# leoelm/Bayesian_inference_for_NN

Measured on NVIDIA B200. Metric: posterior_grad_evals_per_s, higher is better.
Workload: dtype f32 (tensor-core products on two int8 fixed-point slices per operand, kind::i8, exact int32 accumulate; f32 everywhere else)

## Files before the change

bayesian_inference_for_nn_b200/csrc/tc_fused.cuh:

```cuda
#pragma once
#include "tc_layer2.cuh"

namespace pyb {

constexpr int TF_THREADS = 384;
template <int CP> struct TfCfg {
  static constexpr int STAGES = 5;
  static constexpr int W2_BYTES = 2 * 256 * CP * 4;
  static constexpr int ZX_BYTES = 2 * CP * 128 * 4;
  static constexpr int SMEM = STAGES * TP_STAGE_BYTES + 1024  + 1024  + 2048  +
                              128  + W2_BYTES + ZX_BYTES;
  static constexpr int SMEM_I8 = SMEM + 4096;
};
__device__ __forceinline__ void tc_ld_16x256b_x4_raw(uint32_t taddr, uint32_t* r) {
  asm volatile(
      "tcgen05.ld.sync.aligned.16x256b.x4.b32 "
      "{%0, %1, %2, %3, %4, %5, %6, %7, %8, %9, %10, %11, %12, %13, %14, %15}, [%16];"
      : "=r"(r[0]), "=r"(r[1]), "=r"(r[2]), "=r"(r[3]), "=r"(r[4]), "=r"(r[5]), "=r"(r[6]), "=r"(r[7]), "=r"(r[8]),
        "=r"(r[9]), "=r"(r[10]), "=r"(r[11]), "=r"(r[12]), "=r"(r[13]), "=r"(r[14]), "=r"(r[15])
      : "r"(taddr)
      : "memory");
}
__device__ __forceinline__ void tc_mma_i8_pair(uint32_t tmem_d, uint64_t adesc, uint64_t bdesc, uint32_t idesc,
                                               uint32_t accumulate) {
  asm volatile(
      "{\n"
      ".reg .pred p;\n"
      "setp.ne.b32 p, %4, 0;\n"
      "tcgen05.mma.cta_group::2.kind::i8 [%0], %1, %2, %3, p;\n"
      "}\n" ::"r"(tmem_d),
      "l"(adesc), "l"(bdesc), "r"(idesc), "r"(accumulate)
      : "memory");
}
__device__ __forceinline__ void slice4_i8(const float* d, float zq, uint32_t& hw, uint32_t& lw) {
  constexpr float M = 12582912.0f;
  uint32_t hb[4], lb[4];
#pragma unroll
  for (int r = 0; r < 4; ++r) {
    const float t = fmaf(d[r], zq, M);
    const float h = t - M;
    const float e = fmaf(d[r], zq, -h);
    const float u = fmaf(e, 254.0f, M);
    hb[r] = __float_as_uint(t);
    lb[r] = __float_as_uint(u);
  }
  hw = __byte_perm(__byte_perm(hb[0], hb[1], 0x0040), __byte_perm(hb[2], hb[3], 0x0040), 0x5410);
  lw = __byte_perm(__byte_perm(lb[0], lb[1], 0x0040), __byte_perm(lb[2], lb[3], 0x0040), 0x5410);
}

__device__ __forceinline__ void tc_ld_16x256b_x4(uint32_t taddr, float* v) {
  uint32_t r[16];
  asm volatile(
      "tcgen05.ld.sync.aligned.16x256b.x4.b32 "
      "{%0, %1, %2, %3, %4, %5, %6, %7, %8, %9, %10, %11, %12, %13, %14, %15}, [%16];"
      : "=r"(r[0]), "=r"(r[1]), "=r"(r[2]), "=r"(r[3]), "=r"(r[4]), "=r"(r[5]), "=r"(r[6]), "=r"(r[7]), "=r"(r[8]),
        "=r"(r[9]), "=r"(r[10]), "=r"(r[11]), "=r"(r[12]), "=r"(r[13]), "=r"(r[14]), "=r"(r[15])
      : "r"(taddr)
      : "memory");
#pragma unroll
  for (int i = 0; i < 16; ++i) v[i] = __uint_as_float(r[i]);
}
template <int CP>
__device__ __forceinline__ int w2_slot(int h, int c) {
  return ((((h >> 3) * 2 + (h & 1)) * (CP / 4) + (c >> 2)) * 4 + ((h >> 1) & 3)) * 4 + (c & 3);
}
__device__ __forceinline__ void split_pair(float x0, float x1, uint32_t& hw, uint32_t& lw) {
  const __nv_bfloat162 hp = __floats2bfloat162_rn(x0, x1);
  hw = *reinterpret_cast<const uint32_t*>(&hp);
  const __nv_bfloat162 lp = __floats2bfloat162_rn(x0 - __uint_as_float(hw << 16), x1 - __uint_as_float(hw & 0xffff0000u));
  lw = *reinterpret_cast<const uint32_t*>(&lp);
}

template <int CP, bool FWD, int I8 = 0>
__global__ void __cluster_dims__(2, 1, 1) __launch_bounds__(TF_THREADS, 1)
tc_g1_layer2_fused(const __grid_constant__ CUtensorMap tmA_hi, const __grid_constant__ CUtensorMap tmA_lo,
                   const __grid_constant__ CUtensorMap tmB_hi, const __grid_constant__ CUtensorMap tmB_lo,
                   const TcGemmParams p, const Layer2Params l2) {
  constexpr int STAGES = TfCfg<CP>::STAGES;
  extern __shared__ uint8_t smem_raw[];
  uint8_t* smem = smem_raw + ((1024u - (smem_u32(smem_raw) & 1023u)) & 1023u);
  uint8_t* stage_base = smem;
  uint64_t* bars = (uint64_t*)(smem + STAGES * TP_STAGE_BYTES);
  uint64_t* full_bar = bars;
  uint64_t* empty_bar = bars + STAGES;
  uint64_t* tmem_full = bars + 2 * STAGES;
  uint64_t* tmem_empty = bars + 2 * STAGES + 2;
  uint32_t* tmem_ptr = (uint32_t*)(bars + 2 * STAGES + 4);
  float* bias_s = (float*)(smem + STAGES * TP_STAGE_BYTES + 1024);
  float* b2_s = bias_s + 512;
  float* W2_s = b2_s + 32;
  float* zx_s = W2_s + 2 * 256 * CP;
  float* cw_s = zx_s + 2 * CP * 128;
  float* zq_s = cw_s + 512;

  const int warp = __shfl_sync(0xffffffffu, (int)(threadIdx.x >> 5), 0), lane = threadIdx.x & 31;
  const uint32_t rank = cluster_ctarank();
  const int cluster_id = blockIdx.x >> 1, n_clusters = gridDim.x >> 1;
  constexpr int KSTAGE = I8 ? 64 : TC_BK;
  const int nk = (p.K + KSTAGE - 1) / KSTAGE;
  const int H = p.H;
  const int half_rows = H >> 1;
  const uint32_t cta_bytes = 2 * TC_A_TILE_BYTES + 2 * (uint32_t)half_rows * TC_BK * 2;

  if (warp == 8 && lane == 0) {
    asm volatile("prefetch.tensormap [%0];" ::"l"(&tmA_hi) : "memory");
    asm volatile("prefetch.tensormap [%0];" ::"l"(&tmA_lo) : "memory");
    asm volatile("prefetch.tensormap [%0];" ::"l"(&tmB_hi) : "memory");
    asm volatile("prefetch.tensormap [%0];" ::"l"(&tmB_lo) : "memory");
  }
  if (warp == 9 && lane == 0) {
    for (int s = 0; s < STAGES; ++s) { mbar_init(&full_bar[s], 1); mbar_init(&empty_bar[s], 1); }
    mbar_init(&tmem_full[0], 1); mbar_init(&tmem_full[1], 1);
    mbar_init(&tmem_empty[0], 16); mbar_init(&tmem_empty[1], 16);
    asm volatile("fence.mbarrier_init.release.cluster;" ::: "memory");
  }
  if (warp == 10) {
    asm volatile("tcgen05.alloc.cta_group::2.sync.aligned.shared::cta.b32 [%0], %1;" ::"r"(smem_u32(tmem_ptr)), "r"(512)
// ... 47 lines not shown
          tc_fence_after();
          const uint32_t st = smem_u32(stage_base + stage * TP_STAGE_BYTES);
          const int nks = (kc == nk - 1 && k_tail <= KSTAGE / 2) ? 1 : 2;
          for (int ks = 0; ks < nks; ++ks) {
            const uint32_t koff = ks * 32;
            const uint64_t ah = make_smem_desc_sw64(st + koff);
            const uint64_t al = make_smem_desc_sw64(st + TC_A_TILE_BYTES + koff);
            const uint64_t bh = make_smem_desc_sw64(st + 2 * TC_A_TILE_BYTES + koff);
            const uint64_t bl = make_smem_desc_sw64(st + 2 * TC_A_TILE_BYTES + 8192 + koff);
            const uint32_t accum = (kc != 0) || (ks != 0);
            if (I8) {
              tc_mma_i8_pair(d, ah, bh, idesc, accum);
              tc_mma_i8_pair(d + 256, ah, bl, idesc, accum);
              tc_mma_i8_pair(d + 256, al, bh, idesc, 1);
            } else {
              tc_mma_bf16_pair(d, ah, bh, idesc, accum);
              tc_mma_bf16_pair(d, al, bh, idesc, 1);
              tc_mma_bf16_pair(d, ah, bl, idesc, 1);
            }
          }
          tc_commit_pair(&empty_bar[stage]);
          if (++stage == STAGES) { stage = 0; phase ^= 1; }
        }
        tc_commit_pair(&tmem_full[acc]);
      }
    }
   }
  } else {
    asm volatile("setmaxnreg.inc.sync.aligned.u32 232;");
    const int half = warp >> 2;
    const int quad = warp & 3;
    const int g = lane >> 2, t = lane & 3;
    const int eall = threadIdx.x;
    const uint32_t lane_addr = (uint32_t)(quad * 32) << 16;
    const int Hh = H >> 1;
    const int C = l2.C;
    const float invN = l2.scale / (float)l2.N;
    const int r_own = 2 * (t & 1) + (t >> 1);
    const int row_own = quad * 32 + g + 8 * r_own;
    const int pos0 = quad * 32 + 4 * g;
    const int hbase = half * Hh + 2 * t;
    uint16_t* z2_hi = reinterpret_cast<uint16_t*>(l2.z2_hi);
    uint16_t* z2_lo = reinterpret_cast<uint16_t*>(l2.z2_lo);
    for (int i = eall; i < 2 * 256 * CP; i += 256) W2_s[i] = 0.f;
    if (eall < 32) b2_s[eall] = 0.f;
    asm volatile("bar.sync 1, 256;" ::: "memory");
    auto fetch_consts = [&](int item, int buf) {
      int b, mp, split;
      tc_decode(p, item, b, mp, split);
      const float* th = l2.theta + (int64_t)b * l2.P;
      if (eall < H) {
        const int h = eall;
        const float* src = th + l2.w2_off + (int64_t)h * C;
        const uint32_t dst = smem_u32(W2_s + buf * 256 * CP + w2_slot<CP>(h, 0));
#pragma unroll
        for (int c = 0; c < CP; ++c)
          if (c < C)
            asm volatile("cp.async.ca.shared.global [%0], [%1], 4;" ::"r"(dst + (uint32_t)(((c >> 2) * 16 + (c & 3)) * 4)),
                         "l"(src + c) : "memory");
        asm volatile("cp.async.ca.shared.global [%0], [%1], 4;" ::"r"(smem_u32(bias_s + buf * 256 + h)),
                     "l"(p.bias + (int64_t)b * p.bias_stride + h) : "memory");
      }
      if (eall < C)
        asm volatile("cp.async.ca.shared.global [%0], [%1], 4;" ::"r"(smem_u32(b2_s + buf * 16 + eall)),
                     "l"(th + l2.b2_off + eall) : "memory");
      if (I8 && eall < H) {
        asm volatile("cp.async.ca.shared.global [%0], [%1], 4;" ::"r"(smem_u32(cw_s + buf * 256 + eall)),
                     "l"(l2.cw + (int64_t)b * H + eall) : "memory");
        if (I8 == 2 && !FWD)
          asm volatile("cp.async.ca.shared.global [%0], [%1], 4;" ::"r"(smem_u32(zq_s + buf * 256 + eall)),
                       "l"(l2.zq + (int64_t)b * H + eall) : "memory");
      }
    };
    if (cluster_id < p.total_items) fetch_consts(cluster_id, 0);
    int it = 0;
    for (int item = cluster_id; item < p.total_items; item += n_clusters, ++it) {
      int b, mp, split;
      tc_decode(p, item, b, mp, split);
      const int mt = mp * 2 + (int)rank;
      const int cbuf = it & 1;
      const int acc = I8 ? 0 : cbuf;
      const uint32_t acc_phase = I8 ? (uint32_t)(it & 1) : (uint32_t)((it >> 1) & 1);
      float* bs = bias_s + cbuf * 256;
      float* b2b = b2_s + cbuf * 16;
      float* W2b = W2_s + cbuf * 256 * CP;
      float sxr[4] = {0.f, 0.f, 0.f, 0.f};
      if (I8) {
#pragma unroll
        for (int r = 0; r < 4; ++r) {
          const int rg = mt * 128 + quad * 32 + g + 8 * r;
          sxr[r] = rg < p.M_valid ? __ldg(l2.sx + rg) : 0.f;
        }
      }
      asm volatile("cp.async.wait_all;" ::: "memory");
      asm volatile("bar.sync 1, 256;" ::: "memory");
      (I8 ? mbar_wait_sleep(&tmem_full[acc], acc_phase) : mbar_wait(&tmem_full[acc], acc_phase));
      tc_fence_after();
      const int64_t blk_w = (((((int64_t)b * p.out_tiles + mt) * H) + hbase) * 128 + pos0) >> 2;
      uint2* pa_hi = reinterpret_cast<uint2*>(p.out_hi) + blk_w;
      uint2* pa_lo = reinterpret_cast<uint2*>(p.out_lo) + blk_w;
      uint2* pz_hi = reinterpret_cast<uint2*>(l2.zt_hi) + blk_w;
      uint2* pz_lo = reinterpret_cast<uint2*>(l2.zt_lo) + blk_w;
      const float4* w4b = reinterpret_cast<const float4*>(W2b) + (((half * Hh) >> 3) * 2 * (CP / 4)) * 4 + t;
      const float* bsb = bs + hbase;
      const float* cwb = cw_s + cbuf * 256 + hbase;
      const float* zqb = zq_s + cbuf * 256 + hbase;
      uint32_t* pzi_hi = nullptr; uint32_t* pzi_lo = nullptr;
      if (I8 == 2 && !FWD) {
        const int64_t blk_b = ((((int64_t)b * p.out_tiles + mt) * H) + hbase) * 128 + pos0;
        pzi_hi = reinterpret_cast<uint32_t*>(l2.zi_hi + blk_b);
        pzi_lo = reinterpret_cast<uint32_t*>(l2.zi_lo + blk_b);
      }
      float2 z[4][CP / 2];
#pragma unroll
      for (int r = 0; r < 4; ++r)
#pragma unroll
        for (int c = 0; c < CP / 2; ++c) z[r][c] = make_float2(0.f, 0.f);
      uint32_t mask[4] = {0u, 0u, 0u, 0u};
#pragma unroll
      for (int ch = 0; ch < 4; ++ch) {
        if (ch * 32 < Hh) {
          const uint32_t col = (uint32_t)(acc * 256 + half * Hh + ch * 32);
          float v[32];
          if (I8) {
#pragma unroll
            for (int hf = 0; hf < 2; ++hf) {
              uint32_t rh[16], rc[16];
              tc_ld_16x256b_x4_raw(tmem_base + lane_addr + ((uint32_t)(16 * hf) << 16) + col, rh);
              tc_ld_16x256b_x4_raw(tmem_base + lane_addr + ((uint32_t)(16 * hf) << 16) + 256u + col, rc);
              asm volatile("tcgen05.wait::ld.sync.aligned;" ::: "memory");
#pragma unroll
              for (int j = 0; j < 16; ++j)
                v[16 * hf + j] = fmaf((float)(int)rc[j], 1.0f / 254.0f, (float)(int)rh[j]);
            }
          } else {
            tc_ld_16x256b_x4(tmem_base + lane_addr + col, v);
            tc_ld_16x256b_x4(tmem_base + lane_addr + (16u << 16) + col, v + 16);
            asm volatile("tcgen05.wait::ld.sync.aligned;" ::: "memory");
          }
          uint32_t m = 0u;
#pragma unroll
          for (int kb = 0; kb < 4; ++kb) {
            const float2 bb = *reinterpret_cast<const float2*>(bsb + ch * 32 + 8 * kb);
            float2 cc = make_float2(0.f, 0.f);
            if (I8) cc = *reinterpret_cast<const float2*>(cwb + ch * 32 + 8 * kb);
            float a[4][2];
#pragma unroll
            for (int r = 0; r < 4; ++r) {
              const float* vv = v + (r >> 1) * 16 + kb * 4 + (r & 1) * 2;
              if (I8) {
                a[r][0] = fmaxf(fmaf(vv[0], sxr[r] * cc.x, bb.x), 0.f);
                a[r][1] = fmaxf(fmaf(vv[1], sxr[r] * cc.y, bb.y), 0.f);
              } else {
                a[r][0] = fmaxf(vv[0] + bb.x, 0.f);
                a[r][1] = fmaxf(vv[1] + bb.y, 0.f);
              }
              if (!FWD) {
                m |= (a[r][0] > 0.f ? 1u : 0u) << (kb * 8 + r * 2);
                m |= (a[r][1] > 0.f ? 1u : 0u) << (kb * 8 + r * 2 + 1);
              }
            }
#pragma unroll
            for (int i = 0; i < 2; ++i) {
              const float4* w4 = w4b + (((ch * 4 + kb) * 2 + i) * (CP / 4)) * 4;
#pragma unroll
              for (int c4 = 0; c4 < CP / 4; ++c4) {
                const float4 w = w4[c4 * 4];
                const float2 w01 = make_float2(w.x, w.y), w23 = make_float2(w.z, w.w);
#pragma unroll
                for (int r = 0; r < 4; ++r) {
                  const float2 aa = make_float2(a[r][i], a[r][i]);
                  z[r][2 * c4] = __ffma2_rn(aa, w01, z[r][2 * c4]);
                  z[r][2 * c4 + 1] = __ffma2_rn(aa, w23, z[r][2 * c4 + 1]);
                }
              }
              if (!FWD) {
                uint32_t hw0, lw0, hw1, lw1;
                split_pair(a[0][i], a[1][i], hw0, lw0);
                split_pair(a[2][i], a[3][i], hw1, lw1);
                const int w_off = (ch * 32 + 8 * kb + i) * 32;
                __stcs(pa_hi + w_off, make_uint2(hw0, hw1));
                __stcs(pa_lo + w_off, make_uint2(lw0, lw1));
              }
            }
          }
          mask[ch] = m;
        }
      }
      tc_fence_before();
      __syncwarp();
      if (lane == 0) mbar_arrive_leader_relaxed(&tmem_empty[acc]);
      if (item + n_clusters < p.total_items) fetch_consts(item + n_clusters, cbuf ^ 1);
      float zo[CP];
      {
        const bool b0 = t & 1, b1 = t & 2;
#pragma unroll
        for (int c = 0; c < CP; ++c) {
          const float z0 = (c & 1) ? z[0][c >> 1].y : z[0][c >> 1].x, z1 = (c & 1) ? z[1][c >> 1].y : z[1][c >> 1].x;
          const float z2v = (c & 1) ? z[2][c >> 1].y : z[2][c >> 1].x, z3 = (c & 1) ? z[3][c >> 1].y : z[3][c >> 1].x;
          float k0 = b0 ? z2v : z0, k1 = b0 ? z3 : z1;
          const float g0 = __shfl_xor_sync(0xffffffffu, b0 ? z0 : z2v, 1);
          const float g1 = __shfl_xor_sync(0xffffffffu, b0 ? z1 : z3, 1);
          k0 = b0 ? g0 + k0 : k0 + g0;
          k1 = b0 ? g1 + k1 : k1 + g1;
          const float kk = b1 ? k1 : k0;
          const float gg = __shfl_xor_sync(0xffffffffu, b1 ? k0 : k1, 2);
          zo[c] = b1 ? gg + kk : kk + gg;
        }
      }
#pragma unroll
      for (int c = 0; c < CP; ++c) zx_s[(half * CP + c) * 128 + row_own] = zo[c];
      asm volatile("bar.sync 2, 256;" ::: "memory");
      float zf[CP], dz[CP];
#pragma unroll
      for (int c = 0; c < CP; ++c) zf[c] = (b2b[c] + zx_s[c * 128 + row_own]) + zx_s[(CP + c) * 128 + row_own];
      const int row_g = mt * 128 + row_own;
      if (FWD) {
        if (half == 0 && row_g < p.M_valid) {
          float* o = l2.fwd_out + ((int64_t)b * l2.N + row_g) * C;
          if (l2.out_act == PYB_ACT_SOFTMAX) {
            float mx = -INFINITY;
#pragma unroll
            for (int c = 0; c < CP; ++c) if (c < C) mx = fmaxf(mx, zf[c]);
            float se = 0.f;
#pragma unroll
            for (int c = 0; c < CP; ++c) if (c < C) se += expf(zf[c] - mx);
            const float inv = 1.0f / se;
#pragma unroll
            for (int c = 0; c < CP; ++c) if (c < C) o[c] = expf(zf[c] - mx) * inv;
          } else {
#pragma unroll
            for (int c = 0; c < CP; ++c) if (c < C) o[c] = act_apply(zf[c], l2.out_act);
          }
        }
        continue;
      }
      float loss_r = 0.f;
      l2_loss_dz<CP>(l2, row_g, row_g < p.M_valid, zf, dz, loss_r, invN);
      if (half == 0) {
        const int64_t blk2 = (((int64_t)b * p.out_tiles + mt) * L2_CMAX) * 128 + pos0 + r_own;
#pragma unroll
        for (int c = 0; c < CP; ++c) {
          __nv_bfloat16 hb, lb;
          split_bf16(dz[c], hb, lb);
          z2_hi[blk2 + c * 128] = __bfloat16_as_ushort(hb);
          z2_lo[blk2 + c * 128] = __bfloat16_as_ushort(lb);
        }
        const int64_t grp = (int64_t)b * l2.n_groups + mt * 4 + quad;
        float mine = 0.f;
#pragma unroll
        for (int c = 0; c < CP; ++c) {
          const float sm = warp_sum(dz[c]);
          if (lane == c) mine = sm;
        }
        if (lane < CP) l2.b2_partial[grp * L2_CMAX + lane] = mine;
        const float ls = warp_sum(loss_r);
        if (lane == 0) l2.loss_partial[grp] = (double)ls;
      }
      float2 dzp[4][CP / 2];
#pragma unroll
      for (int r = 0; r < 4; ++r) {
        const int src = (lane & ~3) | ((r >> 1) | ((r & 1) << 1));
#pragma unroll
        for (int c = 0; c < CP / 2; ++c) {
          dzp[r][c].x = __shfl_sync(0xffffffffu, dz[2 * c], src);
          dzp[r][c].y = __shfl_sync(0xffffffffu, dz[2 * c + 1], src);
        }
      }
#pragma unroll
      for (int ch = 0; ch < 4; ++ch) {
        if (ch * 32 < Hh) {
          const uint32_t m = mask[ch];
#pragma unroll
          for (int kb = 0; kb < 4; ++kb) {
#pragma unroll
            for (int i = 0; i < 2; ++i) {
              const float4* w4 = w4b + (((ch * 4 + kb) * 2 + i) * (CP / 4)) * 4;
              float2 s[4];
#pragma unroll
              for (int r = 0; r < 4; ++r) s[r] = make_float2(0.f, 0.f);
#pragma unroll
              for (int c4 = 0; c4 < CP / 4; ++c4) {
                const float4 w = w4[c4 * 4];
                const float2 w01 = make_float2(w.x, w.y), w23 = make_float2(w.z, w.w);
#pragma unroll
                for (int r = 0; r < 4; ++r) {
                  s[r] = __ffma2_rn(dzp[r][2 * c4], w01, s[r]);
                  s[r] = __ffma2_rn(dzp[r][2 * c4 + 1], w23, s[r]);
                }
              }
              float d[4];
#pragma unroll
              for (int r = 0; r < 4; ++r) d[r] = ((m >> (kb * 8 + r * 2 + i)) & 1u) ? s[r].x + s[r].y : 0.f;
              const int w_off = (ch * 32 + 8 * kb + i) * 32;
              if (I8 == 2) {
                uint32_t hw, lw;
                slice4_i8(d, zqb[ch * 32 + 8 * kb + i], hw, lw);
                __stcs(pzi_hi + w_off, hw);
                __stcs(pzi_lo + w_off, lw);
              } else {
                uint32_t hw0, lw0, hw1, lw1;
                split_pair(d[0], d[1], hw0, lw0);
                split_pair(d[2], d[3], hw1, lw1);
                __stcs(pz_hi + w_off, make_uint2(hw0, hw1));
                __stcs(pz_lo + w_off, make_uint2(lw0, lw1));
              }
            }
          }
        }
      }
    }
  }
  tc_fence_before();
  __syncthreads();
  cluster_sync_all();
  if (warp == 10) {
    tc_fence_after();
    asm volatile("tcgen05.dealloc.cta_group::2.sync.aligned.b32 %0, %1;" ::"r"(tmem_base), "r"(512) : "memory");
  }
}

}
```

bayesian_inference_for_nn_b200/csrc/tc_layer2.cuh:

```cuda
#pragma once
#include "tc_gemm.cuh"

namespace pyb {

__device__ __forceinline__ void split_bf16(float x, __nv_bfloat16& hi, __nv_bfloat16& lo) {
  hi = __float2bfloat16_rn(x);
  lo = __float2bfloat16_rn(x - __bfloat162float(hi));
}

__global__ void k_split_rows(const float* src, int64_t R, int C, int64_t lds, __nv_bfloat16* hi, __nv_bfloat16* lo,
                             int64_t ldd) {
  const int64_t total = R * C;
  for (int64_t i = (int64_t)blockIdx.x * blockDim.x + threadIdx.x; i < total; i += (int64_t)gridDim.x * blockDim.x) {
    int64_t r = i / C;
    int c = (int)(i - r * C);
    __nv_bfloat16 h, l;
    split_bf16(src[r * lds + c], h, l);
    hi[r * ldd + c] = h;
    lo[r * ldd + c] = l;
  }
}
__global__ void k_split_rows2(const float* __restrict__ src, int64_t R, int C2, int64_t lds, __nv_bfloat16* __restrict__ hi,
                              __nv_bfloat16* __restrict__ lo, int64_t ldd) {
  const int64_t total = R * C2;
// ... 33 lines not shown
  }
}

__global__ void k_fill_ones_perm(__nv_bfloat16* p, int n) {
  for (int i = blockIdx.x * blockDim.x + threadIdx.x; i < n; i += gridDim.x * blockDim.x)
    p[fused_row_pos(i)] = __float2bfloat16_rn(1.0f);
}
__global__ void k_fill_bf16(__nv_bfloat16* p, int64_t n, float v) {
  for (int64_t i = (int64_t)blockIdx.x * blockDim.x + threadIdx.x; i < n; i += (int64_t)gridDim.x * blockDim.x)
    p[i] = __float2bfloat16_rn(v);
}

constexpr int L2_CMAX = 16;
constexpr int L2_ROWS = 256;
struct Layer2Params {
  const __nv_bfloat16* a_hi; const __nv_bfloat16* a_lo;
  __nv_bfloat16* zt_hi; __nv_bfloat16* zt_lo;
  __nv_bfloat16* z2_hi; __nv_bfloat16* z2_lo;
  int k_tiles;
  const float* theta; int64_t P; int64_t w2_off, b2_off;
  int H, C, N, act1, out_act, loss_kind;
  const int32_t* y_i; const float* y_f;
  float scale;
  double* loss_partial;
  float* b2_partial;
  int n_groups, n_tiles;
  float* fwd_out;
  const float* sx;
  const float* cw;
  const float* zq;
  int8_t* zi_hi; int8_t* zi_lo;
  int dbg_flags;
  unsigned long long* dbg;
};
__device__ __forceinline__ float2 unpack_bf16x2(uint32_t v) {
  return make_float2(__uint_as_float(v << 16), __uint_as_float(v & 0xffff0000u));
}
__device__ __forceinline__ uint32_t pack_bf16x2(__nv_bfloat16 a, __nv_bfloat16 b) {
  return (uint32_t)__bfloat16_as_ushort(a) | ((uint32_t)__bfloat16_as_ushort(b) << 16);
}
template <int CP, typename LT>
__device__ __forceinline__ void l2_loss_dz(const Layer2Params& p, int r, bool valid, const float* z, float* dz,
                                           LT& loss_acc, float invN) {
  const int C = p.C;
#pragma unroll
  for (int c = 0; c < CP; ++c) dz[c] = 0.f;
  if (!valid) return;
  if (p.loss_kind == PYB_LOSS_SPARSE_CE) {
    float mx = -INFINITY;
#pragma unroll
    for (int c = 0; c < CP; ++c) if (c < C) mx = fmaxf(mx, z[c]);
    float se = 0.f;
#pragma unroll
    for (int c = 0; c < CP; ++c) if (c < C) se += expf(z[c] - mx);
    const int yi = p.y_i[r];
    float zy = 0.f;
#pragma unroll
    for (int c = 0; c < CP; ++c) if (c == yi) zy = z[c];
    loss_acc += (LT)(logf(se) - (zy - mx));
    const float inv = 1.0f / se;
#pragma unroll
    for (int c = 0; c < CP; ++c)
      if (c < C) dz[c] = (expf(z[c] - mx) * inv - (c == yi ? 1.f : 0.f)) * invN;
  } else {
    float acc = 0.f;
    const float sc = 2.0f * invN / (float)C;
#pragma unroll
    for (int c = 0; c < CP; ++c)
      if (c < C) {
        float a = act_apply(z[c], p.out_act);
        float df = a - p.y_f[(int64_t)r * C + c];
        acc += df * df;
        dz[c] = sc * df * act_grad_from_output(a, p.out_act);
      }
    loss_acc += (LT)(acc / (float)C);
  }
}
template <int CP>
__global__ void __launch_bounds__(128, 4) k_layer2(Layer2Params p) {
  __shared__ __align__(16) float W2s[256 * CP];
  __shared__ float b2s[CP];
  __shared__ uint32_t mask_s[2][8][128];
  __shared__ float redf[4][CP];
  __shared__ double scratch[32];
  const int t = threadIdx.x, b = blockIdx.y;
  const int H = p.H, C = p.C;
  const float* th = p.theta + (int64_t)b * p.P;
  for (int i = t; i < H * CP; i += 128) {
    int h = i / CP, c = i % CP;
    W2s[i] = (c < C) ? th[p.w2_off + (int64_t)h * C + c] : 0.f;
  }
  if (t < CP) b2s[t] = (t < C) ? th[p.b2_off + t] : 0.f;
  __syncthreads();
  const uint32_t* ah = reinterpret_cast<const uint32_t*>(p.a_hi);
  const uint32_t* al = reinterpret_cast<const uint32_t*>(p.a_lo);
  uint32_t* zh = reinterpret_cast<uint32_t*>(p.zt_hi);
  uint32_t* zl = reinterpret_cast<uint32_t*>(p.zt_lo);
  uint32_t* z2h = reinterpret_cast<uint32_t*>(p.z2_hi);
  uint32_t* z2l = reinterpret_cast<uint32_t*>(p.z2_lo);
  const int64_t ld2 = 64;
  float accb[CP];
#pragma unroll
  for (int c = 0; c < CP; ++c) accb[c] = 0.f;
  double loss_acc = 0.0;
  const float invN = p.scale / (float)p.N;
  const bool relu = p.act1 == PYB_ACT_RELU;
  const int nhb = (H + 31) >> 5;
  for (int tile = blockIdx.x; tile < p.n_tiles; tile += gridDim.x) {
    const int r0 = tile * L2_ROWS + 2 * t;
    const int64_t tile128 = (int64_t)b * p.k_tiles + tile * 2 + (t >> 6);
    const int64_t col = tile128 * H * 64 + (t & 63);
    const int64_t col2 = tile128 * L2_CMAX * 64 + (t & 63);
    const bool v0 = r0 < p.N, v1 = r0 + 1 < p.N;
    float z0[CP], z1[CP];
#pragma unroll
    for (int c = 0; c < CP; ++c) { z0[c] = b2s[c]; z1[c] = b2s[c]; }
// ... 204 lines not shown
```

bayesian_inference_for_nn_b200/csrc/tc_path.cu:

```cuda
#include <cstdlib>
#include <cstring>
#include "tc_fused_mma.cuh"
#include <algorithm>

namespace pyb {

typedef CUresult (*PFN_encodeTiled)(CUtensorMap*, CUtensorMapDataType, cuuint32_t, void*, const cuuint64_t*,
                                    const cuuint64_t*, const cuuint32_t*, const cuuint32_t*, CUtensorMapInterleave,
                                    CUtensorMapSwizzle, CUtensorMapL2promotion, CUtensorMapFloatOOBfill);
static PFN_encodeTiled get_encode() {
  static PFN_encodeTiled fn = nullptr;
  if (!fn) {
    void* f = nullptr;
    cudaDriverEntryPointQueryResult q;
    PYB_CUDA(cudaGetDriverEntryPoint("cuTensorMapEncodeTiled", &f, cudaEnableDefault, &q));
    PYB_REQUIRE(f != nullptr && q == cudaDriverEntryPointSuccess, PYB_ERR_CUDA, "cuTensorMapEncodeTiled unavailable");
    fn = (PFN_encodeTiled)f;
  }
  return fn;
}
static CUtensorMap make_map_blocked(const void* base, int64_t blocks, int rows_per_block, int box_rows) {
  CUtensorMap m;
  cuuint64_t dims[3] = {128, (cuuint64_t)rows_per_block, (cuuint64_t)blocks};
  cuuint64_t strides[2] = {256, (cuuint64_t)rows_per_block * 256};
// ... 135 lines not shown
  if ((p.H % 32) != 0) return false;
  return !p.a_blocked && p.a_batch_rows == 0;
}
static void launch_gemm_tc(pyb_handle* h, const CUtensorMap& a_hi, const CUtensorMap& a_lo,
                           const CUtensorMap& b_hi, const CUtensorMap& b_lo, TcGemmParams p, double flops,
                           const CUtensorMap* bp_hi = nullptr, const CUtensorMap* bp_lo = nullptr) {
  if (p.k_splits <= 1) { p.k_splits = 1; p.chunks_per_split = (p.K + TC_BK - 1) / TC_BK; p.split_stride = 0; }
  p.vec_store = p.epi == EPI_STORE && ((uintptr_t)p.out % 16 == 0) && (p.out_stride % 4 == 0) && (p.out_ld % 4 == 0) &&
                (p.split_stride % 4 == 0);
  int grid = std::min(p.total_items, h->sm_count);
  prof_begin(h);
  if (bp_hi && bp_lo && pair_ok(h, p) && p.n_btiles > 1 && p.epi == EPI_STORE && p.transpose_out && h->opt_tc_dual &&
      p.H <= 256 && (p.H / 2) * TC_BK * 2 <= 8192) {
    p.total_items = p.n_batch * p.k_splits * ((p.n_btiles + 1) / 2);
    grid = std::min(2 * p.total_items, (h->sm_count / 2) * 2);
    PYB_CUDA(cudaFuncSetAttribute(tc_gemm_pair_dual_bf16x3, cudaFuncAttributeMaxDynamicSharedMemorySize, TD_SMEM_BYTES));
    tc_gemm_pair_dual_bf16x3<<<grid, TP_THREADS, TD_SMEM_BYTES, h->stream>>>(a_hi, a_lo, *bp_hi, *bp_lo, p);
    prof_end(h, flops);
    count_launch(h);
    return;
  }
  if (bp_hi && bp_lo && pair_ok(h, p)) {
    grid = std::min(2 * p.total_items, (h->sm_count / 2) * 2);
    if (p.epi == EPI_STORE) launch_pair_inst<EPI_STORE, 0>(h, grid, a_hi, a_lo, *bp_hi, *bp_lo, p);
    else if (p.act == PYB_ACT_RELU) launch_pair_inst<EPI_BIAS_ACT_T_SPLIT, PYB_ACT_RELU>(h, grid, a_hi, a_lo, *bp_hi, *bp_lo, p);
    else if (p.act == PYB_ACT_TANH) launch_pair_inst<EPI_BIAS_ACT_T_SPLIT, PYB_ACT_TANH>(h, grid, a_hi, a_lo, *bp_hi, *bp_lo, p);
    else if (p.act == PYB_ACT_SIGMOID) launch_pair_inst<EPI_BIAS_ACT_T_SPLIT, PYB_ACT_SIGMOID>(h, grid, a_hi, a_lo, *bp_hi, *bp_lo, p);
    else launch_pair_inst<EPI_BIAS_ACT_T_SPLIT, PYB_ACT_LINEAR>(h, grid, a_hi, a_lo, *bp_hi, *bp_lo, p);
    prof_end(h, flops);
    count_launch(h);
    return;
  }
  if (p.epi == EPI_STORE) launch_gemm_inst<EPI_STORE, 0>(h, grid, a_hi, a_lo, b_hi, b_lo, p);
  else if (p.act == PYB_ACT_RELU) launch_gemm_inst<EPI_BIAS_ACT_T_SPLIT, PYB_ACT_RELU>(h, grid, a_hi, a_lo, b_hi, b_lo, p);
  else if (p.act == PYB_ACT_TANH) launch_gemm_inst<EPI_BIAS_ACT_T_SPLIT, PYB_ACT_TANH>(h, grid, a_hi, a_lo, b_hi, b_lo, p);
  else if (p.act == PYB_ACT_SIGMOID) launch_gemm_inst<EPI_BIAS_ACT_T_SPLIT, PYB_ACT_SIGMOID>(h, grid, a_hi, a_lo, b_hi, b_lo, p);
  else launch_gemm_inst<EPI_BIAS_ACT_T_SPLIT, PYB_ACT_LINEAR>(h, grid, a_hi, a_lo, b_hi, b_lo, p);
  prof_end(h, flops);
  count_launch(h);
}


template <int CP, bool FWD, int I8>
static void launch_fused_i8(pyb_handle* h, int grid, const CUtensorMap& a_hi, const CUtensorMap& a_lo,
                            const CUtensorMap& b_hi, const CUtensorMap& b_lo, const TcGemmParams& p, const Layer2Params& l2) {
  PYB_CUDA(cudaFuncSetAttribute(tc_g1_layer2_fused<CP, FWD, I8>, cudaFuncAttributeMaxDynamicSharedMemorySize, TfCfg<CP>::SMEM_I8));
  tc_g1_layer2_fused<CP, FWD, I8><<<grid, TF_THREADS, TfCfg<CP>::SMEM_I8, h->stream>>>(a_hi, a_lo, b_hi, b_lo, p, l2);
}
template <int CP>
static void launch_fused_inst(pyb_handle* h, int grid, const CUtensorMap& a_hi, const CUtensorMap& a_lo,
                              const CUtensorMap& b_hi, const CUtensorMap& b_lo, const TcGemmParams& p, const Layer2Params& l2,
                              int i8 = 0) {
  if (i8 && !l2.fwd_out && h->opt_tc_epi_mma) {
    if (i8 >= 2) {
      PYB_CUDA(cudaFuncSetAttribute(tc_fused_i8_mma<CP, true>, cudaFuncAttributeMaxDynamicSharedMemorySize, TfmCfg::SMEM));
      tc_fused_i8_mma<CP, true><<<grid, TFM_THREADS, TfmCfg::SMEM, h->stream>>>(a_hi, a_lo, b_hi, b_lo, p, l2);
    } else {
      PYB_CUDA(cudaFuncSetAttribute(tc_fused_i8_mma<CP, false>, cudaFuncAttributeMaxDynamicSharedMemorySize, TfmCfg::SMEM));
      tc_fused_i8_mma<CP, false><<<grid, TFM_THREADS, TfmCfg::SMEM, h->stream>>>(a_hi, a_lo, b_hi, b_lo, p, l2);
    }
    return;
  }
  if (i8) {
    if (l2.fwd_out) launch_fused_i8<CP, true, 1>(h, grid, a_hi, a_lo, b_hi, b_lo, p, l2);
    else if (i8 >= 2) launch_fused_i8<CP, false, 2>(h, grid, a_hi, a_lo, b_hi, b_lo, p, l2);
    else launch_fused_i8<CP, false, 1>(h, grid, a_hi, a_lo, b_hi, b_lo, p, l2);
    return;
  }
  if (l2.fwd_out) {
    PYB_CUDA(cudaFuncSetAttribute(tc_g1_layer2_fused<CP, true>, cudaFuncAttributeMaxDynamicSharedMemorySize, TfCfg<CP>::SMEM));
    tc_g1_layer2_fused<CP, true><<<grid, TF_THREADS, TfCfg<CP>::SMEM, h->stream>>>(a_hi, a_lo, b_hi, b_lo, p, l2);
    return;
  }
  PYB_CUDA(cudaFuncSetAttribute(tc_g1_layer2_fused<CP, false>, cudaFuncAttributeMaxDynamicSharedMemorySize, TfCfg<CP>::SMEM));
  tc_g1_layer2_fused<CP, false><<<grid, TF_THREADS, TfCfg<CP>::SMEM, h->stream>>>(a_hi, a_lo, b_hi, b_lo, p, l2);
}
static bool fused_ok(const pyb_handle* h, int H, int act1) {
  return h->opt_tc_pair && h->opt_tc_fuse && act1 == PYB_ACT_RELU && (H == 128 || H == 256);
}

static int i8_mode(const pyb_handle* h, bool backward, bool resident) {
  const Model& m = h->model;
  int want = h->opt_tc_i8;
  if (want < 0) want = (resident && backward && h->i8_guard_ok) ? 2 : 0;
  if (want <= 0 || !fused_ok(h, m.layer[0].fan_out, m.layer[0].act) || m.layer[1].fan_out > L2_CMAX) return 0;
  if (m.layer[0].fan_in > 32768) return 0;
  if (!backward) return 1;
  const bool ce = h->loss_kind == PYB_LOSS_SPARSE_CE && m.layer[1].act == PYB_ACT_SOFTMAX;
  return (want >= 2 && ce && m.layer[0].fan_out == 256) ? 2 : 1;
}

static void tc_prepare_data_i8(pyb_handle* h, TcData& d, const float* X, int64_t N, int mode) {
  const int D = d.D;
  const int64_t Npad = d.Npad;
  d.Dk = (D + 15) / 16 * 16;
  d.col_mean.alloc(D); d.col_absmax.alloc(D); d.sx.alloc(N); d.sf.alloc(D + 1);
  d.xs_hi.alloc(N * d.Dk); d.xs_lo.alloc(N * d.Dk);
  d.stat_sum.alloc((size_t)I8_STAT_CHUNKS * D); d.stat_max.alloc((size_t)I8_STAT_CHUNKS * D);
  k_col_stats<<<dim3((D + 31) / 32, I8_STAT_CHUNKS), dim3(32, 32), 0, h->stream>>>(X, N, D, d.stat_sum.p, d.stat_max.p);
  k_col_stats_final<<<(D + 255) / 256, 256, 0, h->stream>>>(d.stat_sum.p, d.stat_max.p, I8_STAT_CHUNKS, N, D, d.col_mean.p,
                                                           d.col_absmax.p);
  count_launch(h);
  const int wpb = 8;
  k_slice_x_rows_i8<<<(unsigned)std::min<int64_t>((N + wpb - 1) / wpb, 8 * (int64_t)h->sm_count), wpb * 32, 0, h->stream>>>(
      X, N, D, d.col_mean.p, d.xs_hi.p, d.xs_lo.p, d.sx.p, d.Dk);
  count_launch(h, 2);
  d.mXs_hi = make_map_u8p(d.xs_hi.p, d.Dk, N, d.Dk, 128);
  d.mXs_lo = make_map_u8p(d.xs_lo.p, d.Dk, N, d.Dk, 128);
  if (mode >= 2) {
    d.xts_hi.alloc((int64_t)(D + 1) * Npad); d.xts_lo.alloc((int64_t)(D + 1) * Npad);
    PYB_CUDA(cudaMemsetAsync(d.xts_hi.p, 0, (size_t)(D + 1) * Npad, h->stream));
    PYB_CUDA(cudaMemsetAsync(d.xts_lo.p, 0, (size_t)(D + 1) * Npad, h->stream));
// ... 94 lines not shown
    st->ws_hi.alloc(cc * H * Dk); st->ws_lo.alloc(cc * H * Dk);
    st->cw.alloc(cc * H); st->b1c.alloc(cc * H); st->zq.alloc(cc * H); st->zd.alloc(cc * H);
    st->mWs_hi = make_map_u8p(st->ws_hi.p, Dk, cc * H, Dk, H / 2);
    st->mWs_lo = make_map_u8p(st->ws_lo.p, Dk, cc * H, Dk, H / 2);
    if (mode >= 2) {
      st->cap_blocks_i8 = std::max(st->cap_blocks_i8, need_blocks);
      const int64_t cb = st->cap_blocks_i8;
      st->zi_hi.alloc(cb * H * 128); st->zi_lo.alloc(cb * H * 128);
      st->mZi_hi = make_map_blocked_u8(st->zi_hi.p, cb, H, 128);
      st->mZi_lo = make_map_blocked_u8(st->zi_lo.p, cb, H, 128);
    }
  }
  return bc;
}

static void tc_pack_and_g1(pyb_handle* h, TcState* st, TcData& d, const float* th, int nb,
                           const Layer2Params* fused = nullptr, int i8 = 0) {
  const Model& m = h->model;
  const LayerDesc& L1 = m.layer[0];
  const int D = st->D, H = st->H;
  const int64_t N = d.N, Npad = d.Npad, P = m.P;
  if (i8) {
    const float invN = fused->fwd_out ? 1.0f : fused->scale / (float)fused->N;
    k_pack_w1_i8<<<dim3((H + 31) / 32, nb), dim3(32, 8), 0, h->stream>>>(
        th, P, L1.w_off, L1.b_off, m.layer[1].w_off, D, H, m.layer[1].fan_out, d.col_mean.p, invN, st->ws_hi.p, st->ws_lo.p,
        d.Dk, st->cw.p, st->b1c.p, st->zq.p, st->zd.p);
  } else {
  dim3 g((H + 31) / 32, (D + 31) / 32, nb), blk(32, 8);
  k_split_transpose<<<g, blk, 0, h->stream>>>(th + L1.w_off, P, D, H, H, st->w_hi.p, st->w_lo.p, (int64_t)H * D, D);
  }
  count_launch(h);
  TcGemmParams p = {};
  p.K = D; p.n_mtiles = (int)(Npad / 128); p.n_pairs = (p.n_mtiles + 1) / 2; p.n_batch = nb; p.H = H;
  p.a_batch_rows = 0; p.a_box_rows = 128; p.order = 1; p.sub_batch = 32; p.total_items = p.n_pairs * nb;
  p.epi = EPI_BIAS_ACT_T_SPLIT;
  p.bias = th + L1.b_off; p.bias_stride = P; p.act = L1.act;
  p.out_hi = st->a_hi.p; p.out_lo = st->a_lo.p; p.out_tiles = (int)(Npad / 128);
  p.M_valid = (int)N; p.N_valid = H;
  if (fused) {
    const int grid = std::min(2 * p.total_items, (h->sm_count / 2) * 2);
    const int C = fused->C;
    Layer2Params f2 = *fused;
    const CUtensorMap &a_hi = i8 ? d.mXs_hi : d.mX_hi, &a_lo = i8 ? d.mXs_lo : d.mX_lo;
    const CUtensorMap &b_hi = i8 ? st->mWs_hi : st->mWp_hi, &b_lo = i8 ? st->mWs_lo : st->mWp_lo;
    if (i8) {
      p.bias = st->b1c.p; p.bias_stride = H;
      f2.dbg = nullptr; f2.dbg_flags = h->opt_tc_timeline & ~1;
      if (h->opt_tc_timeline) { st->dbg.alloc(8 * 160); f2.dbg = st->dbg.p; }
      f2.sx = d.sx.p; f2.cw = st->cw.p; f2.zq = st->zq.p; f2.zi_hi = st->zi_hi.p; f2.zi_lo = st->zi_lo.p;
    }
    prof_begin(h);
    if (C <= 4) launch_fused_inst<4>(h, grid, a_hi, a_lo, b_hi, b_lo, p, f2, i8);
    else if (C <= 8) launch_fused_inst<8>(h, grid, a_hi, a_lo, b_hi, b_lo, p, f2, i8);
    else if (C <= 12) launch_fused_inst<12>(h, grid, a_hi, a_lo, b_hi, b_lo, p, f2, i8);
    else launch_fused_inst<16>(h, grid, a_hi, a_lo, b_hi, b_lo, p, f2, i8);
    prof_end(h, 2.0 * N * (D * (double)H + (fused->fwd_out ? 1.0 : 3.0) * H * C) * nb);
    count_launch(h);
    return;
  }
  launch_gemm_tc(h, d.mX_hi, d.mX_lo, st->mW_hi, st->mW_lo, p, 2.0 * N * D * (double)H * nb, &st->mWp_hi, &st->mWp_lo);
}

static void tc_eval_on(pyb_handle* h, TcState* st, TcData& d, const int32_t* y_i, const float* y_f, const float* theta,
                       int64_t S, float scale, float* loss_out, float* grad_out) {
  const Model& m = h->model;
  const int64_t Bc = tc_prepare_bufs(h, st, S, d.Npad, true, d.i8);
  const LayerDesc& L1 = m.layer[0];
  const LayerDesc& L2 = m.layer[1];
  const int D = st->D, H = st->H, C = st->C;
  const int64_t N = d.N, Npad = d.Npad, P = m.P;
  const int n_tiles = (int)(Npad / L2_ROWS);
  const bool fused = fused_ok(h, H, L1.act) && C <= L2_CMAX;
  const int i8 = d.i8;
  const int n_groups = fused ? (int)(Npad / 128) * 4
                             : std::min(n_tiles, std::max(1, (int)((8 * (int64_t)h->sm_count + Bc - 1) / Bc)));
  st->b2_partial.alloc((size_t)Bc * n_groups * L2_CMAX);
  st->loss_partial.alloc((size_t)Bc * n_groups);
  for (int64_t b0 = 0; b0 < S; b0 += Bc) {
    const int nb = (int)std::min<int64_t>(Bc, S - b0);
    const float* th = theta + b0 * P;
    float* gr = grad_out + b0 * P;
    {
      Layer2Params p = {};
      p.a_hi = st->a_hi.p; p.a_lo = st->a_lo.p; p.zt_hi = st->z_hi.p; p.zt_lo = st->z_lo.p;
      p.z2_hi = st->z2_hi.p; p.z2_lo = st->z2_lo.p; p.k_tiles = (int)(Npad / 128);
      p.theta = th; p.P = P; p.w2_off = L2.w_off; p.b2_off = L2.b_off;
      p.H = H; p.C = C; p.N = (int)N; p.act1 = L1.act; p.out_act = L2.act; p.loss_kind = h->loss_kind;
      p.y_i = y_i; p.y_f = y_f; p.scale = scale;
      p.loss_partial = st->loss_partial.p; p.b2_partial = st->b2_partial.p; p.n_groups = n_groups;
      p.n_tiles = n_tiles;
      if (fused) {
        tc_pack_and_g1(h, st, d, th, nb, &p, i8);
      } else {
        tc_pack_and_g1(h, st, d, th, nb);
        dim3 g(n_groups, nb);
        if (C <= 4) k_layer2<4><<<g, 128, 0, h->stream>>>(p);
        else if (C <= 8) k_layer2<8><<<g, 128, 0, h->stream>>>(p);
        else if (C <= 12) k_layer2<12><<<g, 128, 0, h->stream>>>(p);
        else k_layer2<16><<<g, 128, 0, h->stream>>>(p);
      }
      k_layer2_reduce<<<nb, 256, 0, h->stream>>>(st->b2_partial.p, st->loss_partial.p, n_groups, C, gr, P, L2.b_off,
                                                loss_out ? loss_out + b0 : nullptr, (int)N);
      count_launch(h, 2);
    }
    const int nk_rows = (int)(Npad / TC_BK);
    const int splits = (nk_rows + TC_SPLIT_CHUNKS - 1) / TC_SPLIT_CHUNKS;
// ... 288 lines not shown
```

Measured before the change: 10760.

## Add CP=10 class padding and split layer-2 epilogue across halves

```diff
diff --git a/bayesian_inference_for_nn_b200/csrc/tc_fused.cuh b/bayesian_inference_for_nn_b200/csrc/tc_fused.cuh
--- a/bayesian_inference_for_nn_b200/csrc/tc_fused.cuh
+++ b/bayesian_inference_for_nn_b200/csrc/tc_fused.cuh
@@ -6,6 +6,7 @@
 constexpr int TF_THREADS = 384;
 template <int CP> struct TfCfg {
   static constexpr int STAGES = 5;
+  static_assert(CP % 2 == 0 && CP <= 16, "even class padding, at most L2_CMAX classes");
   static constexpr int W2_BYTES = 2 * 256 * CP * 4;
   static constexpr int ZX_BYTES = 2 * CP * 128 * 4;
   static constexpr int SMEM = STAGES * TP_STAGE_BYTES + 1024  + 1024  + 2048  +
@@ -62,7 +63,10 @@
 }
 template <int CP>
 __device__ __forceinline__ int w2_slot(int h, int c) {
-  return ((((h >> 3) * 2 + (h & 1)) * (CP / 4) + (c >> 2)) * 4 + ((h >> 1) & 3)) * 4 + (c & 3);
+  static_assert(CP % 2 == 0, "the class padding is even");
+  constexpr int CP4 = CP / 4 * 4;
+  const int grp = ((h >> 3) * 2 + (h & 1)) * 4 * CP, t = (h >> 1) & 3;
+  return grp + (c < CP4 ? ((c >> 2) * 4 + t) * 4 + (c & 3) : 4 * CP4 + 2 * t + (c - CP4));
 }
 __device__ __forceinline__ void split_pair(float x0, float x1, uint32_t& hw, uint32_t& lw) {
   const __nv_bfloat162 hp = __floats2bfloat162_rn(x0, x1);
@@ -216,11 +220,11 @@
       if (eall < H) {
         const int h = eall;
         const float* src = th + l2.w2_off + (int64_t)h * C;
-        const uint32_t dst = smem_u32(W2_s + buf * 256 * CP + w2_slot<CP>(h, 0));
+        float* dst = W2_s + buf * 256 * CP;
 #pragma unroll
         for (int c = 0; c < CP; ++c)
           if (c < C)
-            asm volatile("cp.async.ca.shared.global [%0], [%1], 4;" ::"r"(dst + (uint32_t)(((c >> 2) * 16 + (c & 3)) * 4)),
+            asm volatile("cp.async.ca.shared.global [%0], [%1], 4;" ::"r"(smem_u32(dst + w2_slot<CP>(h, c))),
                          "l"(src + c) : "memory");
         asm volatile("cp.async.ca.shared.global [%0], [%1], 4;" ::"r"(smem_u32(bias_s + buf * 256 + h)),
                      "l"(p.bias + (int64_t)b * p.bias_stride + h) : "memory");
@@ -265,7 +269,10 @@
       uint2* pa_lo = reinterpret_cast<uint2*>(p.out_lo) + blk_w;
       uint2* pz_hi = reinterpret_cast<uint2*>(l2.zt_hi) + blk_w;
       uint2* pz_lo = reinterpret_cast<uint2*>(l2.zt_lo) + blk_w;
-      const float4* w4b = reinterpret_cast<const float4*>(W2b) + (((half * Hh) >> 3) * 2 * (CP / 4)) * 4 + t;
+      constexpr int CP4 = CP / 4 * 4;
+      const float* w2h = W2b + ((half * Hh) >> 3) * 2 * 4 * CP;
+      const float4* w4b = reinterpret_cast<const float4*>(w2h) + t;
+      const float2* w2b = reinterpret_cast<const float2*>(w2h + 4 * CP4) + t;
       const float* bsb = bs + hbase;
       const float* cwb = cw_s + cbuf * 256 + hbase;
       const float* zqb = zq_s + cbuf * 256 + hbase;
@@ -326,7 +333,8 @@
             }
 #pragma unroll
             for (int i = 0; i < 2; ++i) {
-              const float4* w4 = w4b + (((ch * 4 + kb) * 2 + i) * (CP / 4)) * 4;
+              const int grp = (ch * 4 + kb) * 2 + i;
+              const float4* w4 = w4b + grp * CP;
 #pragma unroll
               for (int c4 = 0; c4 < CP / 4; ++c4) {
                 const float4 w = w4[c4 * 4];
@@ -337,6 +345,11 @@
                   z[r][2 * c4] = __ffma2_rn(aa, w01, z[r][2 * c4]);
                   z[r][2 * c4 + 1] = __ffma2_rn(aa, w23, z[r][2 * c4 + 1]);
                 }
+              }
+              if (CP != CP4) {
+                const float2 w = w2b[grp * 2 * CP];
+#pragma unroll
+                for (int r = 0; r < 4; ++r) z[r][CP / 2 - 1] = __ffma2_rn(make_float2(a[r][i], a[r][i]), w, z[r][CP / 2 - 1]);
               }
               if (!FWD) {
                 uint32_t hw0, lw0, hw1, lw1;
@@ -375,33 +388,43 @@
 #pragma unroll
       for (int c = 0; c < CP; ++c) zx_s[(half * CP + c) * 128 + row_own] = zo[c];
       asm volatile("bar.sync 2, 256;" ::: "memory");
-      float zf[CP], dz[CP];
-#pragma unroll
-      for (int c = 0; c < CP; ++c) zf[c] = (b2b[c] + zx_s[c * 128 + row_own]) + zx_s[(CP + c) * 128 + row_own];
       const int row_g = mt * 128 + row_own;
-      if (FWD) {
-        if (half == 0 && row_g < p.M_valid) {
-          float* o = l2.fwd_out + ((int64_t)b * l2.N + row_g) * C;
-          if (l2.out_act == PYB_ACT_SOFTMAX) {
-            float mx = -INFINITY;
-#pragma unroll
-            for (int c = 0; c < CP; ++c) if (c < C) mx = fmaxf(mx, zf[c]);
-            float se = 0.f;
-#pragma unroll
-            for (int c = 0; c < CP; ++c) if (c < C) se += expf(zf[c] - mx);
-            const float inv = 1.0f / se;
-#pragma unroll
-            for (int c = 0; c < CP; ++c) if (c < C) o[c] = expf(zf[c] - mx) * inv;
-          } else {
-#pragma unroll
-            for (int c = 0; c < CP; ++c) if (c < C) o[c] = act_apply(zf[c], l2.out_act);
+      float dz[CP];
+      if (half == 0) {
+        float zf[CP];
+#pragma unroll
+        for (int c = 0; c < CP; ++c) zf[c] = (b2b[c] + zx_s[c * 128 + row_own]) + zx_s[(CP + c) * 128 + row_own];
+        if (FWD) {
+          if (row_g < p.M_valid) {
+            float* o = l2.fwd_out + ((int64_t)b * l2.N + row_g) * C;
+            if (l2.out_act == PYB_ACT_SOFTMAX) {
+              float mx = -INFINITY;
+#pragma unroll
+              for (int c = 0; c < CP; ++c) if (c < C) mx = fmaxf(mx, zf[c]);
+              float se = 0.f;
+#pragma unroll
+              for (int c = 0; c < CP; ++c) if (c < C) { dz[c] = expf(zf[c] - mx); se += dz[c]; }
+              const float inv = 1.0f / se;
+#pragma unroll
+              for (int c = 0; c < CP; ++c) if (c < C) o[c] = dz[c] * inv;
+            } else {
+#pragma unroll
+              for (int c = 0; c < CP; ++c) if (c < C) o[c] = act_apply(zf[c], l2.out_act);
+            }
           }
-        }
-        continue;
-      }
-      float loss_r = 0.f;
-      l2_loss_dz<CP>(l2, row_g, row_g < p.M_valid, zf, dz, loss_r, invN);
-      if (half == 0) {
+        } else {
+          float loss_r = 0.f;
+          l2_loss_dz<CP>(l2, row_g, row_g < p.M_valid, zf, dz, loss_r, invN);
+#pragma unroll
+          for (int c = 0; c < CP; ++c) zx_s[c * 128 + row_own] = dz[c];
+          asm volatile("bar.arrive 3, 256;" ::: "memory");
+          const float ls = warp_sum(loss_r);
+          if (lane == 0) l2.loss_partial[(int64_t)b * l2.n_groups + mt * 4 + quad] = (double)ls;
+        }
+      } else if (!FWD) {
+        asm volatile("bar.sync 3, 256;" ::: "memory");
+#pragma unroll
+        for (int c = 0; c < CP; ++c) dz[c] = zx_s[c * 128 + row_own];
         const int64_t blk2 = (((int64_t)b * p.out_tiles + mt) * L2_CMAX) * 128 + pos0 + r_own;
 #pragma unroll
         for (int c = 0; c < CP; ++c) {
@@ -418,9 +441,8 @@
           if (lane == c) mine = sm;
         }
         if (lane < CP) l2.b2_partial[grp * L2_CMAX + lane] = mine;
-        const float ls = warp_sum(loss_r);
-        if (lane == 0) l2.loss_partial[grp] = (double)ls;
-      }
+      }
+      if (FWD) continue;
       float2 dzp[4][CP / 2];
 #pragma unroll
       for (int r = 0; r < 4; ++r) {
@@ -439,7 +461,8 @@
           for (int kb = 0; kb < 4; ++kb) {
 #pragma unroll
             for (int i = 0; i < 2; ++i) {
-              const float4* w4 = w4b + (((ch * 4 + kb) * 2 + i) * (CP / 4)) * 4;
+              const int grp = (ch * 4 + kb) * 2 + i;
+              const float4* w4 = w4b + grp * CP;
               float2 s[4];
 #pragma unroll
               for (int r = 0; r < 4; ++r) s[r] = make_float2(0.f, 0.f);
@@ -452,6 +475,11 @@
                   s[r] = __ffma2_rn(dzp[r][2 * c4], w01, s[r]);
                   s[r] = __ffma2_rn(dzp[r][2 * c4 + 1], w23, s[r]);
                 }
+              }
+              if (CP != CP4) {
+                const float2 w = w2b[grp * 2 * CP];
+#pragma unroll
+                for (int r = 0; r < 4; ++r) s[r] = __ffma2_rn(dzp[r][CP / 2 - 1], w, s[r]);
               }
               float d[4];
 #pragma unroll
diff --git a/bayesian_inference_for_nn_b200/csrc/tc_layer2.cuh b/bayesian_inference_for_nn_b200/csrc/tc_layer2.cuh
--- a/bayesian_inference_for_nn_b200/csrc/tc_layer2.cuh
+++ b/bayesian_inference_for_nn_b200/csrc/tc_layer2.cuh
@@ -109,7 +109,7 @@
     for (int c = 0; c < CP; ++c) if (c < C) mx = fmaxf(mx, z[c]);
     float se = 0.f;
 #pragma unroll
-    for (int c = 0; c < CP; ++c) if (c < C) se += expf(z[c] - mx);
+    for (int c = 0; c < CP; ++c) if (c < C) { dz[c] = expf(z[c] - mx); se += dz[c]; }
     const int yi = p.y_i[r];
     float zy = 0.f;
 #pragma unroll
@@ -118,7 +118,7 @@
     const float inv = 1.0f / se;
 #pragma unroll
     for (int c = 0; c < CP; ++c)
-      if (c < C) dz[c] = (expf(z[c] - mx) * inv - (c == yi ? 1.f : 0.f)) * invN;
+      if (c < C) dz[c] = (dz[c] * inv - (c == yi ? 1.f : 0.f)) * invN;
   } else {
     float acc = 0.f;
     const float sc = 2.0f * invN / (float)C;
diff --git a/bayesian_inference_for_nn_b200/csrc/tc_path.cu b/bayesian_inference_for_nn_b200/csrc/tc_path.cu
--- a/bayesian_inference_for_nn_b200/csrc/tc_path.cu
+++ b/bayesian_inference_for_nn_b200/csrc/tc_path.cu
@@ -211,12 +211,13 @@
                               const CUtensorMap& b_hi, const CUtensorMap& b_lo, const TcGemmParams& p, const Layer2Params& l2,
                               int i8 = 0) {
   if (i8 && !l2.fwd_out && h->opt_tc_epi_mma) {
+    constexpr int CPM = (CP + 3) / 4 * 4;
     if (i8 >= 2) {
-      PYB_CUDA(cudaFuncSetAttribute(tc_fused_i8_mma<CP, true>, cudaFuncAttributeMaxDynamicSharedMemorySize, TfmCfg::SMEM));
-      tc_fused_i8_mma<CP, true><<<grid, TFM_THREADS, TfmCfg::SMEM, h->stream>>>(a_hi, a_lo, b_hi, b_lo, p, l2);
+      PYB_CUDA(cudaFuncSetAttribute(tc_fused_i8_mma<CPM, true>, cudaFuncAttributeMaxDynamicSharedMemorySize, TfmCfg::SMEM));
+      tc_fused_i8_mma<CPM, true><<<grid, TFM_THREADS, TfmCfg::SMEM, h->stream>>>(a_hi, a_lo, b_hi, b_lo, p, l2);
     } else {
-      PYB_CUDA(cudaFuncSetAttribute(tc_fused_i8_mma<CP, false>, cudaFuncAttributeMaxDynamicSharedMemorySize, TfmCfg::SMEM));
-      tc_fused_i8_mma<CP, false><<<grid, TFM_THREADS, TfmCfg::SMEM, h->stream>>>(a_hi, a_lo, b_hi, b_lo, p, l2);
+      PYB_CUDA(cudaFuncSetAttribute(tc_fused_i8_mma<CPM, false>, cudaFuncAttributeMaxDynamicSharedMemorySize, TfmCfg::SMEM));
+      tc_fused_i8_mma<CPM, false><<<grid, TFM_THREADS, TfmCfg::SMEM, h->stream>>>(a_hi, a_lo, b_hi, b_lo, p, l2);
     }
     return;
   }
@@ -417,6 +418,7 @@
     prof_begin(h);
     if (C <= 4) launch_fused_inst<4>(h, grid, a_hi, a_lo, b_hi, b_lo, p, f2, i8);
     else if (C <= 8) launch_fused_inst<8>(h, grid, a_hi, a_lo, b_hi, b_lo, p, f2, i8);
+    else if (C <= 10) launch_fused_inst<10>(h, grid, a_hi, a_lo, b_hi, b_lo, p, f2, i8);
     else if (C <= 12) launch_fused_inst<12>(h, grid, a_hi, a_lo, b_hi, b_lo, p, f2, i8);
     else launch_fused_inst<16>(h, grid, a_hi, a_lo, b_hi, b_lo, p, f2, i8);
     prof_end(h, 2.0 * N * (D * (double)H + (fused->fwd_out ? 1.0 : 3.0) * H * C) * nb);
```

New measurement: 10940 (median of 6 runs). 1.6% higher.
